# ComparativeGenomicsToolkit/paffy

Measured on AMD Instinct MI355X. Metric: PAF records/sec (shatter+invert+trim pipe); % HBM roofline at 1/2/4/8 GPU, higher is better.
Workload: dtype u8/int64 (float32 identity predicate); 1 GPU; cfg3: 10M synthetic PAF records, mean 2k cigar ops, invert | trim | shatter; pipe=invert|trim|shatter, pipeline_contexts=2, stream_records=10000000, mean_cigar_ops=2048

## Files before the change

### paffy_amd/csrc/flat_kernel.h

```cpp
#ifndef PAFFY_FLAT_KERNEL_H_
#define PAFFY_FLAT_KERNEL_H_

#define FLAT_TILE 1024u
#define FLAT_TILE_SHIFT 10u
#define FLAT_CHUNK_PIECES 4u
#define FLAT_P_CAP 512u
#define FLAT_NO_CHUNK 0xffffffffu
#define FLAT_F_IRREG 1u
#define FLAT_F_NONPLAIN 2u

struct PieceSum {
    uint32_t cnt;
    uint32_t m, x;
    uint32_t ins, del;
    uint32_t rows;
    uint32_t extra;
    uint32_t text_end;
};
static_assert(sizeof(PieceSum) == 32, "two 16-byte stores");

struct FlatParams {
    const uint8_t *in;
    uint32_t in_len;
    const RecMeta *meta;
    const uint32_t *chunk_rec;
    uint32_t n_chunk_slots;
    const uint16_t *nd;
    PieceSum *sums;
    uint32_t *ops_mirror;
    DevInfo *info;
    uint32_t items_mode;
};

__device__ __forceinline__ uint32_t nondigit16(const uint4 &v) {
    const uint32_t w[4] = {v.x, v.y, v.z, v.w};
    uint32_t m = 0;
#pragma unroll
    for (int j = 0; j < 4; j++) {
        uint32_t nd = nondigit4(w[j]) >> 7;
        nd = (nd | (nd >> 7) | (nd >> 14) | (nd >> 21)) & 0xfu;
        m |= nd << (4 * j);
    }
    return m;
}
__device__ __forceinline__ uint32_t wave_fold_u32(uint32_t x) {
    x += dpp_mov_u32<DPP_ROW_SHR(1), 0xf, 0xf>(x);
    x += dpp_mov_u32<DPP_ROW_SHR(2), 0xf, 0xf>(x);
    x += dpp_mov_u32<DPP_ROW_SHR(4), 0xf, 0xf>(x);
    x += dpp_mov_u32<DPP_ROW_SHR(8), 0xf, 0xf>(x);
    x += dpp_mov_u32<DPP_BCAST15, 0xa, 0xf>(x);
    x += dpp_mov_u32<DPP_BCAST31, 0xc, 0xf>(x);
    return x;
}
__device__ __forceinline__ uint32_t wave_sum_u32(uint32_t v) { return wave_last_u32(wave_fold_u32(v)); }
__device__ __forceinline__ void wave_sum6_u32(uint32_t (&x)[6]) {
#define FLAT_FOLD_STEP(CTRL, RM)                                                  \
    _Pragma("unroll") for (int k = 0; k < 6; k++) x[k] += dpp_mov_u32<CTRL, RM, 0xf>(x[k]);
    FLAT_FOLD_STEP(DPP_ROW_SHR(1), 0xf)
    FLAT_FOLD_STEP(DPP_ROW_SHR(2), 0xf)
    FLAT_FOLD_STEP(DPP_ROW_SHR(4), 0xf)
    FLAT_FOLD_STEP(DPP_ROW_SHR(8), 0xf)
    FLAT_FOLD_STEP(DPP_BCAST15, 0xa)
    FLAT_FOLD_STEP(DPP_BCAST31, 0xc)
#undef FLAT_FOLD_STEP
#pragma unroll
    for (int k = 0; k < 6; k++) x[k] = wave_last_u32(x[k]);
}
__device__ __forceinline__ uint32_t uni(uint32_t x) { return (uint32_t)__builtin_amdgcn_readfirstlane((int)x); }
__device__ __forceinline__ uint32_t lane_val(uint32_t x, uint32_t l) { return (uint32_t)__builtin_amdgcn_readlane((int)x, (int)l); }

#define FLAT_PARSE_LDS (16u + FLAT_TILE + 2u * FLAT_P_CAP)
#define FLAT_PARSE_WAVES 4u
template <uint32_t MODE>
__global__ __launch_bounds__(64 * FLAT_PARSE_WAVES) void k_flat_parse(FlatParams F) {
    __shared__ __attribute__((aligned(16))) uint8_t smem[FLAT_PARSE_WAVES][FLAT_PARSE_LDS];
    const uint32_t lane = threadIdx.x & 63u, wave = uni(threadIdx.x >> 6);
    uint8_t *T = smem[wave];
    uint16_t *Pl = reinterpret_cast<uint16_t *>(T + 16u + FLAT_TILE);
    const uint32_t n_waves = gridDim.x * FLAT_PARSE_WAVES;
    for (uint32_t c = blockIdx.x * FLAT_PARSE_WAVES + wave; c < F.n_chunk_slots; c += n_waves) {
        const uint32_t rec = F.chunk_rec[c];
        if (rec == FLAT_NO_CHUNK) continue;
        const uint32_t cg_off = F.meta[rec].cg_off, cg_end = cg_off + F.meta[rec].cg_len;
        const uint32_t tile_first = cg_off >> FLAT_TILE_SHIFT;
        const uint32_t np = ((cg_end - 1u) >> FLAT_TILE_SHIFT) - tile_first + 1u;
        const uint32_t p0 = (c - ((tile_first >> 2) + rec)) * FLAT_CHUNK_PIECES, p1 = p0 + FLAT_CHUNK_PIECES < np ? p0 + FLAT_CHUNK_PIECES : np;
        PieceSum *const rec_sums = F.sums + (tile_first + rec);
        uint32_t tile = tile_first + p0;
        __builtin_amdgcn_wave_barrier();
        if (lane == 0) {
            uint4 h = make_uint4(0, 0, 0, 0);
            if (tile > 0) h = *reinterpret_cast<const uint4 *>(F.in + ((size_t)tile << FLAT_TILE_SHIFT) - 16u);
            *reinterpret_cast<uint4 *>(T) = h;
        }
        __builtin_amdgcn_wave_barrier();
        uint32_t n = 0;
        int32_t prev;
        uint32_t text_end = 0;
        if (p0 == 0) {
            prev = (int32_t)cg_off - 1 - (int32_t)(tile << FLAT_TILE_SHIFT);
        } else {
            uint32_t cnt = 0;
            {
                const uint32_t g = (tile_first << FLAT_TILE_SHIFT) + lane * 16u;
                uint4 v = make_uint4(0x30303030u, 0x30303030u, 0x30303030u, 0x30303030u);
                if (g < F.in_len) v = *reinterpret_cast<const uint4 *>(F.in + g);
                const uint32_t lo_b = cg_off > g ? (cg_off - g < 16u ? cg_off - g : 16u) : 0u;
                cnt = (uint32_t)__popc(nondigit16(v) & 0xffffu & ~((1u << lo_b) - 1u));
            }
            for (uint32_t t = tile_first + 1u + lane; t < tile; t += 64u) cnt += F.nd[t];
            n = wave_sum_u32(cnt);
            const uint4 h = *reinterpret_cast<const uint4 *>(T);
            const uint32_t hm = nondigit16(h);
            prev = hm ? (int32_t)(31 - __clz((int)hm)) - 16 : -17;
            text_end = (uint32_t)((int32_t)(tile << FLAT_TILE_SHIFT) + prev + 1 - (int32_t)cg_off);
        }
        uint16_t *dst = reinterpret_cast<uint16_t *>(F.ops_mirror + (cg_off >> 1));
        for (uint32_t p = p0; p < p1; p++, tile++) {
            const uint32_t t0 = tile << FLAT_TILE_SHIFT, g = t0 + lane * 16u;
            uint4 v = make_uint4(0, 0, 0, 0);
            if (g < F.in_len) v = *reinterpret_cast<const uint4 *>(F.in + g);
            *reinterpret_cast<uint4 *>(T + 16u + lane * 16u) = v;
            const uint32_t ndm = nondigit16(v);
            const uint32_t lo_b = cg_off > g ? (cg_off - g < 16u ? cg_off - g : 16u) : 0u;
            const uint32_t hi_b = cg_end < g + 16u ? (cg_end > g ? cg_end - g : 0u) : 16u;
            uint32_t opmask = ndm & (hi_b >= 16u ? 0xffffu : ((1u << hi_b) - 1u)) & ~((1u << lo_b) - 1u);
            uint32_t bad = (hi_b > lo_b && g + hi_b == cg_end && !((ndm >> (hi_b - 1u)) & 1u)) ? 1u : 0u;
            const uint32_t cnt = (uint32_t)__popc(opmask), inc = wave_incl_scan_u32(cnt), total = wave_last_u32(inc);
            uint32_t rank = inc - cnt;
            while (opmask) {
                const uint32_t j = (uint32_t)__ffs((int)opmask) - 1u;
                opmask &= opmask - 1u;
                if (rank < FLAT_P_CAP) Pl[rank] = (uint16_t)(lane * 16u + j);
                rank++;
            }
            if (total > FLAT_P_CAP) bad = 1u;
            __builtin_amdgcn_wave_barrier();
            const uint32_t top = total < FLAT_P_CAP ? total : FLAT_P_CAP;
            uint32_t acc_mx = 0, acc_id = 0, acc_re = 0, nonplain = 0;
            uint32_t before_first = (uint32_t)prev;
            for (uint32_t i = lane; i < top; i += 64u) {
                const uint32_t pos = Pl[i];
                const uint32_t before = (uint32_t)__builtin_amdgcn_update_dpp((int)before_first, (int)pos, 0x138 , 0xf, 0xf, false);
                before_first = lane_val(pos, 63);
                const uint32_t k = pos - before - 1u;
                const uint32_t a = 12u + pos, sh = a & 3u;
                const uint32_t *wp = reinterpret_cast<const uint32_t *>(T + (a - sh));
                const uint32_t d0 = wp[0], d1 = wp[1];
                const uint32_t hi = __builtin_amdgcn_alignbyte(d1, d0, sh);
                const uint32_t ch = (d1 >> (8u * sh)) & 0xffu;
                const uint32_t kk = k < 4u ? k : 4u;
                const uint32_t x = kk ? ((hi ^ 0x30303030u) & (0xffffffffu << (32u - 8u * kk))) : 0u;
                const uint32_t pr = ((x << 3) + (x << 1) + (x >> 8)) & 0x00ff00ffu;
                const uint32_t len = __umul24(pr & 0xffu, 100u) + (pr >> 16);
                const uint32_t dl = ch - 0x3du;
                const bool known = dl < 28u && ((0x08011081u >> dl) & 1u);
                const uint32_t code = (0x04001023u >> (dl & 0x1cu)) & 7u;
                const bool lead0 = kk >= 2u && ((hi >> (8u * (4u - kk))) & 0xffu) == (uint32_t)'0';
                bad |= ((k - 1u > 3u) | (len - 1u >= 8191u) | lead0 | !known) ? 1u : 0u;
                dst[n + i] = (uint16_t)((len << 3) | code);
                const uint32_t l16 = len & 0xffffu;
                acc_mx += l16 << (((0x16u >> code) & 1u) << 4);
                acc_id += (code == (uint32_t)OP_I ? l16 : 0u) + (code == (uint32_t)OP_D ? l16 << 16 : 0u);
                if (MODE == 2u) acc_re += (code == (uint32_t)OP_M ? 1u : 0u) + (code == (uint32_t)OP_I ? 1u << 16 : 0u);
                else acc_re += code == (uint32_t)OP_M ? 1u + ((MODE == 1u ? (len + 15u) >> 4 : kk - 1u) << 16) : 0u;
                nonplain |= code > (uint32_t)OP_D ? 1u : 0u;
            }
            uint32_t sums6[6] = {acc_mx & 0xffffu, acc_mx >> 16, acc_id & 0xffffu, acc_id >> 16, acc_re & 0xffffu, acc_re >> 16};
            wave_sum6_u32(sums6);
            const uint32_t s_m = sums6[0], s_x = sums6[1], s_i = sums6[2], s_d = sums6[3], s_r = sums6[4], s_e = sums6[5];
            const uint32_t flags = (__any(bad != 0) ? FLAT_F_IRREG : 0u) | (__any(nonplain != 0) ? FLAT_F_NONPLAIN : 0u);
            if (total) {
                const int32_t last = (int32_t)Pl[top - 1u];
                text_end = t0 + (uint32_t)last + 1u - cg_off;
                prev = last - (int32_t)FLAT_TILE;
            } else {
                prev -= (int32_t)FLAT_TILE;
                if (prev < -64) prev = -64;
            }
            if (lane == 0) {
                uint4 *o = reinterpret_cast<uint4 *>(rec_sums + p);
                o[0] = make_uint4(total | (flags << 16), s_m, s_x, s_i);
                o[1] = make_uint4(s_d, s_r, s_e, text_end);
            }
            n += total;
            __builtin_amdgcn_wave_barrier();
            if (lane == 63u) *reinterpret_cast<uint4 *>(T) = v;
            __builtin_amdgcn_wave_barrier();
        }
    }
}


struct FlatSizeParams {
    KParams P;
    PieceSum *sums;
    uint8_t *flat_done;
    uint32_t *defer;
};

struct FlatPre {
    uint32_t cnt, m, x, ins, del, rows, extra, text;
};
__device__ __forceinline__ FlatPre flat_sub(const FlatPre &a, const FlatPre &b) {
    FlatPre r;
    r.cnt = a.cnt - b.cnt; r.m = a.m - b.m; r.x = a.x - b.x; r.ins = a.ins - b.ins; r.del = a.del - b.del;
    r.rows = a.rows - b.rows; r.extra = a.extra - b.extra; r.text = a.text - b.text;
    return r;
}
__device__ __forceinline__ uint32_t flat_ld(const uint32_t *p) { return __hip_atomic_load(p, __ATOMIC_RELAXED, __HIP_MEMORY_SCOPE_AGENT); }

struct FlatRec {
    const PieceSum *ps;
    uint32_t np, n_ops;
    bool in_regs;
    FlatPre inc;
    const uint16_t *ops;
    bool want_text;
    bool extra_icount;

    __device__ __forceinline__ FlatPre piece_prefix(uint32_t j) const {
        FlatPre r;
        r.cnt = r.m = r.x = r.ins = r.del = r.rows = r.extra = r.text = 0;
        if (j == 0) return r;
        if (in_regs) {
            const uint32_t l = j - 1u;
            r.cnt = lane_val(inc.cnt, l); r.m = lane_val(inc.m, l); r.x = lane_val(inc.x, l); r.ins = lane_val(inc.ins, l);
            r.del = lane_val(inc.del, l); r.rows = lane_val(inc.rows, l); r.extra = lane_val(inc.extra, l); r.text = lane_val(inc.text, l);
        } else {
            const uint32_t *q = reinterpret_cast<const uint32_t *>(ps + (j - 1u));
            r.cnt = uni(flat_ld(q)); r.m = uni(flat_ld(q + 1)); r.x = uni(flat_ld(q + 2)); r.ins = uni(flat_ld(q + 3));
            r.del = uni(flat_ld(q + 4)); r.rows = uni(flat_ld(q + 5)); r.extra = uni(flat_ld(q + 6)); r.text = uni(flat_ld(q + 7));
        }
        return r;
    }
    __device__ __forceinline__ uint32_t piece_of(uint32_t r) const {
        if (in_regs) {
            const uint32_t lane = threadIdx.x & 63u;
            return (uint32_t)__popcll(__ballot(lane < np && inc.cnt <= r));
        }
        uint32_t lo = 0, hi = np;
        while (lo < hi) {
            const uint32_t mid = (lo + hi) >> 1;
            if (uni(flat_ld(&ps[mid].cnt)) <= r) lo = mid + 1u;
            else hi = mid;
        }
        return lo;
    }
    __device__ __forceinline__ FlatPre raw_prefix(uint32_t r) const {
        if (r >= n_ops) return piece_prefix(np);
        const uint32_t pc = piece_of(r);
        FlatPre a = piece_prefix(pc);
        if (a.cnt == r) return a;
        const uint32_t lane = threadIdx.x & 63u;
        uint32_t sm = 0, sx = 0, si = 0, sd = 0, sr = 0, se = 0, st = 0;
        for (uint32_t i = a.cnt + lane; i < r; i += 64u) {
            const uint32_t w = ops[i], len = w >> 3, code = w & 7u;
            const uint32_t is_m = 0u - ((0x9u >> code) & 1u);
            const uint32_t dg = (len >= 10u) + (len >= 100u) + (len >= 1000u);
            sm += len & is_m;
            sx += len & ~is_m;
            si += code == (uint32_t)OP_I ? len : 0u;
            sd += code == (uint32_t)OP_D ? len : 0u;
            sr += code == (uint32_t)OP_M ? 1u : 0u;
            se += extra_icount ? (code == (uint32_t)OP_I ? 1u : 0u) : (code == (uint32_t)OP_M ? dg : 0u);
            st += dg + 2u;
        }
        uint32_t sums6[6] = {sm, sx, si, sd, sr, se};
        wave_sum6_u32(sums6);
        a.m += sums6[0]; a.x += sums6[1]; a.ins += sums6[2]; a.del += sums6[3];
        a.rows += sums6[4]; a.extra += sums6[5];
        if (want_text) a.text += wave_sum_u32(st);
        a.cnt = r;
        return a;
    }
};

struct FlatView {
    uint32_t lo, n;
    bool rev, swp;
    FlatPre wlo, whi;
    uint32_t cut_m = 0, cut_x = 0;
    __device__ __forceinline__ uint32_t tm() const { return whi.m - wlo.m - cut_m; }
    __device__ __forceinline__ uint32_t tx() const { return whi.x - wlo.x - cut_x; }
    __device__ __forceinline__ uint32_t ins_v() const { return swp ? whi.del - wlo.del : whi.ins - wlo.ins; }
    __device__ __forceinline__ uint32_t del_v() const { return swp ? whi.ins - wlo.ins : whi.del - wlo.del; }
    __device__ __forceinline__ int64_t tq() const { return (int64_t)tm() + (int64_t)tx() - (int64_t)del_v(); }
    __device__ __forceinline__ int64_t tt() const { return (int64_t)tm() + (int64_t)tx() - (int64_t)ins_v(); }
};

struct FlatState {
    int64_t qlen, qs, qe, tlen, ts, te;
    bool same;
};
__device__ __forceinline__ void flat_invert(FlatState &s) {
    int64_t t;
    t = s.qs; s.qs = s.ts; s.ts = t;
    t = s.qe; s.qe = s.te; s.te = t;
    t = s.qlen; s.qlen = s.tlen; s.tlen = t;
}
__device__ __forceinline__ int flat_check(const FlatState &s, const FlatView &v) {
    if (s.qs < 0 || s.qs >= s.qlen) return PAFFY_ERR_CHECK_QSTART;
    if (s.qs > s.qe || s.qe > s.qlen) return PAFFY_ERR_CHECK_QEND;
    if (s.ts < 0 || s.ts >= s.tlen) return PAFFY_ERR_CHECK_TSTART;
    if (s.ts > s.te || s.te > s.tlen) return PAFFY_ERR_CHECK_TEND;
    if (v.tq() != s.qe - s.qs) return PAFFY_ERR_CHECK_CIGAR_Q;
    if (v.tt() != s.te - s.ts) return PAFFY_ERR_CHECK_CIGAR_T;
    return 0;
}

__device__ __forceinline__ bool flat_filter_pass(const KParams &P, const RecMeta &m, const FlatView &v) {
    const int64_t mm = v.tm(), mx = v.tx();
    const int64_t all = mm + mx;
    const int64_t ins = all - v.tt(), del = all - v.tq();
    const double identity = ratio_f32(mm, mm + (mx - ins - del));
    const double identity_with_gaps = ratio_f32(mm, all);
    const int64_t f_as = P.filter.min_alignment_score, f_cs = P.filter.min_chain_score, f_tl = P.filter.max_tile_level;
    const double f_id = P.filter.min_identity, f_idg = P.filter.min_identity_with_gaps;
    return m.score >= f_as && m.chain_score >= f_cs && (f_tl == -1 || m.tile_level <= f_tl) && identity >= f_id && identity_with_gaps >= f_idg;
}
__device__ __forceinline__ void flat_dropped(const KParams &P, uint8_t *flat_done, uint32_t rec) {
    RecPlan *dp = static_cast<RecPlan *>(P.rec_plan) + rec;
    flat_done[rec] = 1;
    P.status[rec] = (uint32_t)KLASS_LDS << 16;
    P.err_aux[rec] = 0;
    P.n_ops[rec] = 0;
    P.out_len[rec] = 0;
    P.out_rows[rec] = 0;
    dp->flags = 128u;
    dp->n = 0;
}

__device__ __forceinline__ void flat_stats(const KParams &P, uint32_t rec, const FlatView &v) {
    const uint32_t n_i = v.whi.extra - v.wlo.extra, n_other = (v.whi.cnt - v.wlo.cnt) - (v.whi.rows - v.wlo.rows);
    const uint32_t n_d = n_other - n_i;
    int64_t *o = P.rec_stats + 6ull * rec;
    o[0] = (int64_t)v.tm();
    o[1] = (int64_t)v.tx() - (int64_t)(v.whi.ins - v.wlo.ins) - (int64_t)(v.whi.del - v.wlo.del);
    o[2] = (int64_t)(v.swp ? n_d : n_i);
    o[3] = (int64_t)(v.swp ? n_i : n_d);
    o[4] = (int64_t)v.ins_v();
    o[5] = (int64_t)v.del_v();
}
__device__ __forceinline__ bool flat_ratio_lt(uint32_t num, uint32_t den, float thr_f, double thr) {
    const float nf = __uint2float_rn(num), df = __uint2float_rn(den);
    const float p = __fmul_rn(thr_f, df);
    if (nf < __fmul_rn(p, 0.999996f)) return true;
    if (nf > __fmul_rn(p, 1.000004f)) return false;
    return (double)__fdiv_rn(nf, df) < thr;
}
__device__ __forceinline__ bool flat_ratio_ge(uint32_t num, uint32_t den, float id_f, double idd) {
    const float nf = __uint2float_rn(num), df = __uint2float_rn(den);
    const float p = __fmul_rn(id_f, df);
    if (nf > __fmul_rn(p, 1.000004f)) return true;
    if (nf < __fmul_rn(p, 0.999996f)) return false;
    return (double)__fdiv_rn(nf, df) >= idd;
}

__device__ __forceinline__ void flat_trim_prefix(const FlatRec &R, FlatState &s, FlatView &v, float thr_f, float id_f, int64_t max_trim) {
    const double thr = (double)thr_f, idd = (double)id_f;
    const uint32_t lane = threadIdx.x & 63u;
    const uint32_t w_end = v.lo + v.n;
    const uint32_t nb = (R.np + 63u) >> 6;
    int32_t trim_idx = -1;
    uint32_t hit_m = 0, hit_x = 0;
    for (uint32_t bi = 0; bi < nb && trim_idx < 0; bi++) {
        const uint32_t b = v.rev ? bi : nb - 1u - bi;
        const uint32_t p = b * 64u + lane;
        uint32_t a_cnt = 0, a_m = 0, a_x = 0, b_cnt = 0, b_m = 0, b_x = 0;
        if (p < R.np) {
            if (R.in_regs) {
                b_cnt = R.inc.cnt; b_m = R.inc.m; b_x = R.inc.x;
            } else {
                const uint32_t *q = reinterpret_cast<const uint32_t *>(R.ps + p);
                b_cnt = flat_ld(q); b_m = flat_ld(q + 1); b_x = flat_ld(q + 2);
            }
        }
        if (R.in_regs) {
            a_cnt = dpp_mov_u32<0x138, 0xf, 0xf>(b_cnt); a_m = dpp_mov_u32<0x138, 0xf, 0xf>(b_m); a_x = dpp_mov_u32<0x138, 0xf, 0xf>(b_x);
        } else if (p > 0 && p < R.np) {
            const uint32_t *q = reinterpret_cast<const uint32_t *>(R.ps + (p - 1u));
            a_cnt = flat_ld(q); a_m = flat_ld(q + 1); a_x = flat_ld(q + 2);
        }
        if (a_cnt < v.lo) { a_cnt = v.lo; a_m = v.wlo.m; a_x = v.wlo.x; }
        if (a_cnt > w_end) { a_cnt = w_end; a_m = v.whi.m; a_x = v.whi.x; }
        if (b_cnt < v.lo) { b_cnt = v.lo; b_m = v.wlo.m; b_x = v.wlo.x; }
        if (b_cnt > w_end) { b_cnt = w_end; b_m = v.whi.m; b_x = v.whi.x; }
        const bool live = p < R.np && b_cnt > a_cnt;
        const uint32_t c_m = v.rev ? v.whi.m - b_m : a_m - v.wlo.m, c_x = v.rev ? v.whi.x - b_x : a_x - v.wlo.x;
        const uint32_t chunk_x = b_x - a_x;
        const bool may_hit = live && !(c_m > 0 && (double)c_m >= thr * 1.00001 * (double)(c_m + c_x + chunk_x)) &&
                             !(max_trim >= 0 && (int64_t)c_m + (int64_t)c_x > max_trim);
        unsigned long long flagged = __ballot(may_hit);
        while (flagged) {
            const uint32_t t = v.rev ? (uint32_t)__ffsll((long long)flagged) - 1u : 63u - (uint32_t)__clzll((long long)flagged);
            flagged &= ~(1ull << t);
            const uint32_t ra = lane_val(a_cnt, t), rb = lane_val(b_cnt, t);
            uint32_t pm = lane_val(c_m, t), px = lane_val(c_x, t);
            const uint32_t x_end = px + lane_val(chunk_x, t);
            const uint32_t vb = v.rev ? w_end - rb : ra - v.lo, ve = v.rev ? w_end - ra : rb - v.lo;
            int32_t hit = -1;
            for (uint32_t i0 = vb; i0 < ve; i0 += 64u) {
                if (i0 != vb && pm > 0 && (double)pm >= thr * 1.00001 * (double)(pm + x_end)) break;
                const uint32_t i = i0 + lane;
                uint32_t len = 0, code = 0;
                if (i < ve) {
                    const uint32_t w = R.ops[v.rev ? w_end - 1u - i : v.lo + i];
                    len = w >> 3;
                    code = w & 7u;
                }
                const uint32_t is_m = 0u - ((0x9u >> code) & 1u);
                const uint32_t im = wave_incl_scan_u32(len & is_m), ix = wave_incl_scan_u32(len & ~is_m);
                const uint32_t cm = pm + im, cx = px + ix;
                const bool ok = i < ve && !(max_trim >= 0 && (int64_t)(cm + cx) > max_trim) && flat_ratio_lt(cm, cm + cx, thr_f, thr);
                const unsigned long long hb = __ballot(ok);
                if (hb) {
                    const uint32_t hl = 63u - (uint32_t)__clzll((long long)hb);
                    hit = (int32_t)(i0 + hl);
                    hit_m = lane_val(cm, hl);
                    hit_x = lane_val(cx, hl);
                }
                pm += wave_last_u32(im);
                px += wave_last_u32(ix);
            }
            if (hit >= 0) {
                trim_idx = hit;
                break;
            }
        }
    }
    if (trim_idx < 0) return;
    uint32_t best = 0xffffffffu;
    {
        uint32_t pm = 0, px = 0;
        for (uint32_t i0 = 0; i0 <= (uint32_t)trim_idx && best == 0xffffffffu; i0 += 64u) {
            const uint32_t i = i0 + lane;
            uint32_t len = 0, code = 0;
            if (i <= (uint32_t)trim_idx) {
                const uint32_t w = R.ops[v.rev ? w_end - 1u - i : v.lo + i];
                len = w >> 3;
                code = w & 7u;
            }
            const uint32_t is_m = 0u - ((0x9u >> code) & 1u);
            const uint32_t vm = len & is_m, vx = len & ~is_m;
            const uint32_t im = wave_incl_scan_u32(vm), ix = wave_incl_scan_u32(vx);
            const uint32_t sm = hit_m - (pm + im - vm), sx = hit_x - (px + ix - vx);
            const bool ok = i <= (uint32_t)trim_idx && flat_ratio_ge(sm, sm + sx, id_f, idd);
            const unsigned long long hb = __ballot(ok);
            if (hb) best = i0 + (uint32_t)__ffsll((long long)hb) - 1u;
            pm += wave_last_u32(im);
            px += wave_last_u32(ix);
        }
    }
    const uint32_t count = best != 0xffffffffu ? best : (uint32_t)trim_idx + 1u;
    if (count == 0) return;
    const int64_t old_tt = v.tt(), old_tq = v.tq();
    {
        const FlatPre cut = R.raw_prefix(v.rev ? v.lo + v.n - count : v.lo + count);
        if (v.rev) {
            v.whi = cut;
        } else {
            v.wlo = cut;
            v.lo += count;
        }
    }
    v.n -= count;
    const int64_t d_t = old_tt - v.tt(), d_q = old_tq - v.tq();
    s.ts += d_t;
    if (s.same) s.qs += d_q;
    else s.qe -= d_q;
}

#define FLAT_F_ROW_PIECES 0x200000u
#define FLAT_F_COPY 0x400000u
#define FLAT_COPY_MAX (1u << 18)
#define FLAT_ROW_PIECES_BYTES 144u
// ... 947 lines not shown
```

Baseline: 24.72 million records/s.

## Rewrite flat-parse CIGAR decode with udot4 digit math and LDS-absolute op positions

Replaces the per-byte nondigit mask fold with udot4 dot products, and stores absolute LDS byte addresses in the op-position list so the previous op position is read from memory instead of a DPP shift plus readlane. CIGAR length decoding uses udot4. Validity checks are OR-accumulated into three bitmasks and tested once after the loop. Per-op accumulators are trimmed: the X sum is rebuilt as I+D, and =/X ops go through a wave-uniform slow path with a separate reduction. The position list grows to a full tile and output stores use global address-space pointers. This cuts VALU work in the decode loop, at the cost of more LDS and subtle invariants about address encoding and validity equivalence.

```diff
diff --git a/paffy_amd/csrc/flat_kernel.h b/paffy_amd/csrc/flat_kernel.h
--- a/paffy_amd/csrc/flat_kernel.h
+++ b/paffy_amd/csrc/flat_kernel.h
@@ -32,16 +32,11 @@
     uint32_t items_mode;
 };
 
+__device__ __forceinline__ uint32_t udot4(uint32_t x, uint32_t w, uint32_t a) { return __builtin_amdgcn_udot4(x, w, a, false); }
 __device__ __forceinline__ uint32_t nondigit16(const uint4 &v) {
-    const uint32_t w[4] = {v.x, v.y, v.z, v.w};
-    uint32_t m = 0;
-#pragma unroll
-    for (int j = 0; j < 4; j++) {
-        uint32_t nd = nondigit4(w[j]) >> 7;
-        nd = (nd | (nd >> 7) | (nd >> 14) | (nd >> 21)) & 0xfu;
-        m |= nd << (4 * j);
-    }
-    return m;
+    const uint32_t lo = udot4(nondigit4(v.y), 0x80402010u, udot4(nondigit4(v.x), 0x08040201u, 0u));
+    const uint32_t hi = udot4(nondigit4(v.w), 0x80402010u, udot4(nondigit4(v.z), 0x08040201u, 0u));
+    return (hi << 1) | (lo >> 7);
 }
 __device__ __forceinline__ uint32_t wave_fold_u32(uint32_t x) {
     x += dpp_mov_u32<DPP_ROW_SHR(1), 0xf, 0xf>(x);
@@ -53,9 +48,10 @@
     return x;
 }
 __device__ __forceinline__ uint32_t wave_sum_u32(uint32_t v) { return wave_last_u32(wave_fold_u32(v)); }
-__device__ __forceinline__ void wave_sum6_u32(uint32_t (&x)[6]) {
+template <int N>
+__device__ __forceinline__ void wave_sums_u32(uint32_t (&x)[N]) {
 #define FLAT_FOLD_STEP(CTRL, RM)                                                  \
-    _Pragma("unroll") for (int k = 0; k < 6; k++) x[k] += dpp_mov_u32<CTRL, RM, 0xf>(x[k]);
+    _Pragma("unroll") for (int k = 0; k < N; k++) x[k] += dpp_mov_u32<CTRL, RM, 0xf>(x[k]);
     FLAT_FOLD_STEP(DPP_ROW_SHR(1), 0xf)
     FLAT_FOLD_STEP(DPP_ROW_SHR(2), 0xf)
     FLAT_FOLD_STEP(DPP_ROW_SHR(4), 0xf)
@@ -64,19 +60,27 @@
     FLAT_FOLD_STEP(DPP_BCAST31, 0xc)
 #undef FLAT_FOLD_STEP
 #pragma unroll
-    for (int k = 0; k < 6; k++) x[k] = wave_last_u32(x[k]);
-}
+    for (int k = 0; k < N; k++) x[k] = wave_last_u32(x[k]);
+}
+__device__ __forceinline__ void wave_sum6_u32(uint32_t (&x)[6]) { wave_sums_u32<6>(x); }
 __device__ __forceinline__ uint32_t uni(uint32_t x) { return (uint32_t)__builtin_amdgcn_readfirstlane((int)x); }
 __device__ __forceinline__ uint32_t lane_val(uint32_t x, uint32_t l) { return (uint32_t)__builtin_amdgcn_readlane((int)x, (int)l); }
 
-#define FLAT_PARSE_LDS (16u + FLAT_TILE + 2u * FLAT_P_CAP)
+#define FLAT_P_SLOTS FLAT_TILE
+#define FLAT_PARSE_PL (16u + FLAT_TILE + 16u)
+#define FLAT_PARSE_LDS (FLAT_PARSE_PL + 2u * FLAT_P_SLOTS)
 #define FLAT_PARSE_WAVES 4u
+#define FLAT_CODE_TAB 0x34770127u
+#define FLAT_CODE_LETTERS_LO 0x3d44494du
+#define FLAT_CODE_LETTERS_HI 0xffffff58u
 template <uint32_t MODE>
 __global__ __launch_bounds__(64 * FLAT_PARSE_WAVES) void k_flat_parse(FlatParams F) {
     __shared__ __attribute__((aligned(16))) uint8_t smem[FLAT_PARSE_WAVES][FLAT_PARSE_LDS];
     const uint32_t lane = threadIdx.x & 63u, wave = uni(threadIdx.x >> 6);
+    uint8_t *const L = &smem[0][0];
     uint8_t *T = smem[wave];
-    uint16_t *Pl = reinterpret_cast<uint16_t *>(T + 16u + FLAT_TILE);
+    const uint32_t ebase = wave * FLAT_PARSE_LDS + 12u;
+    const uint32_t pl0 = wave * FLAT_PARSE_LDS + FLAT_PARSE_PL;
     const uint32_t n_waves = gridDim.x * FLAT_PARSE_WAVES;
     for (uint32_t c = blockIdx.x * FLAT_PARSE_WAVES + wave; c < F.n_chunk_slots; c += n_waves) {
         const uint32_t rec = F.chunk_rec[c];
@@ -115,7 +119,9 @@
             prev = hm ? (int32_t)(31 - __clz((int)hm)) - 16 : -17;
             text_end = (uint32_t)((int32_t)(tile << FLAT_TILE_SHIFT) + prev + 1 - (int32_t)cg_off);
         }
-        uint16_t *dst = reinterpret_cast<uint16_t *>(F.ops_mirror + (cg_off >> 1));
+        const uintptr_t dst = reinterpret_cast<uintptr_t>(F.ops_mirror + (cg_off >> 1)) - (uintptr_t)(pl0 - 2u);
+        typedef __attribute__((address_space(1))) uint8_t *GlobalBytes;
+        typedef __attribute__((address_space(1))) uint16_t *GlobalWord;
         for (uint32_t p = p0; p < p1; p++, tile++) {
             const uint32_t t0 = tile << FLAT_TILE_SHIFT, g = t0 + lane * 16u;
             uint4 v = make_uint4(0, 0, 0, 0);
@@ -127,51 +133,71 @@
             uint32_t opmask = ndm & (hi_b >= 16u ? 0xffffu : ((1u << hi_b) - 1u)) & ~((1u << lo_b) - 1u);
             uint32_t bad = (hi_b > lo_b && g + hi_b == cg_end && !((ndm >> (hi_b - 1u)) & 1u)) ? 1u : 0u;
             const uint32_t cnt = (uint32_t)__popc(opmask), inc = wave_incl_scan_u32(cnt), total = wave_last_u32(inc);
-            uint32_t rank = inc - cnt;
-            while (opmask) {
-                const uint32_t j = (uint32_t)__ffs((int)opmask) - 1u;
-                opmask &= opmask - 1u;
-                if (rank < FLAT_P_CAP) Pl[rank] = (uint16_t)(lane * 16u + j);
-                rank++;
+            {
+                uint32_t w = pl0 + 2u * (inc - cnt);
+                const uint32_t e0 = ebase + lane * 16u;
+                for (; opmask; opmask &= opmask - 1u, w += 2u) *reinterpret_cast<uint16_t *>(L + w) = (uint16_t)(e0 + (uint32_t)__builtin_ctz(opmask));
+                if (lane == 0) *reinterpret_cast<int16_t *>(L + pl0 - 2u) = (int16_t)((int32_t)ebase + (prev < -17 ? -17 : prev));
             }
             if (total > FLAT_P_CAP) bad = 1u;
             __builtin_amdgcn_wave_barrier();
             const uint32_t top = total < FLAT_P_CAP ? total : FLAT_P_CAP;
-            uint32_t acc_mx = 0, acc_id = 0, acc_re = 0, nonplain = 0;
-            uint32_t before_first = (uint32_t)prev;
-            for (uint32_t i = lane; i < top; i += 64u) {
-                const uint32_t pos = Pl[i];
-                const uint32_t before = (uint32_t)__builtin_amdgcn_update_dpp((int)before_first, (int)pos, 0x138 , 0xf, 0xf, false);
-                before_first = lane_val(pos, 63);
-                const uint32_t k = pos - before - 1u;
-                const uint32_t a = 12u + pos, sh = a & 3u;
-                const uint32_t *wp = reinterpret_cast<const uint32_t *>(T + (a - sh));
-                const uint32_t d0 = wp[0], d1 = wp[1];
-                const uint32_t hi = __builtin_amdgcn_alignbyte(d1, d0, sh);
-                const uint32_t ch = (d1 >> (8u * sh)) & 0xffu;
-                const uint32_t kk = k < 4u ? k : 4u;
-                const uint32_t x = kk ? ((hi ^ 0x30303030u) & (0xffffffffu << (32u - 8u * kk))) : 0u;
-                const uint32_t pr = ((x << 3) + (x << 1) + (x >> 8)) & 0x00ff00ffu;
-                const uint32_t len = __umul24(pr & 0xffu, 100u) + (pr >> 16);
-                const uint32_t dl = ch - 0x3du;
-                const bool known = dl < 28u && ((0x08011081u >> dl) & 1u);
-                const uint32_t code = (0x04001023u >> (dl & 0x1cu)) & 7u;
-                const bool lead0 = kk >= 2u && ((hi >> (8u * (4u - kk))) & 0xffu) == (uint32_t)'0';
-                bad |= ((k - 1u > 3u) | (len - 1u >= 8191u) | lead0 | !known) ? 1u : 0u;
-                dst[n + i] = (uint16_t)((len << 3) | code);
-                const uint32_t l16 = len & 0xffffu;
-                acc_mx += l16 << (((0x16u >> code) & 1u) << 4);
-                acc_id += (code == (uint32_t)OP_I ? l16 : 0u) + (code == (uint32_t)OP_D ? l16 << 16 : 0u);
-                if (MODE == 2u) acc_re += (code == (uint32_t)OP_M ? 1u : 0u) + (code == (uint32_t)OP_I ? 1u << 16 : 0u);
-                else acc_re += code == (uint32_t)OP_M ? 1u + ((MODE == 1u ? (len + 15u) >> 4 : kk - 1u) << 16) : 0u;
-                nonplain |= code > (uint32_t)OP_D ? 1u : 0u;
-            }
-            uint32_t sums6[6] = {acc_mx & 0xffffu, acc_mx >> 16, acc_id & 0xffffu, acc_id >> 16, acc_re & 0xffffu, acc_re >> 16};
-            wave_sum6_u32(sums6);
-            const uint32_t s_m = sums6[0], s_x = sums6[1], s_i = sums6[2], s_d = sums6[3], s_r = sums6[4], s_e = sums6[5];
-            const uint32_t flags = (__any(bad != 0) ? FLAT_F_IRREG : 0u) | (__any(nonplain != 0) ? FLAT_F_NONPLAIN : 0u);
+            uint32_t v_len = 0, v_dig = 0, v_let = 0;
+            uint32_t acc_m = 0;
+            uint32_t acc_id = 0;
+            uint32_t acc_r = 0;
+            uint32_t acc_eq = 0, acc_xx = 0;
+            uint32_t eqx = 0;
+            const uint32_t a_end = pl0 - 2u + 2u * top;
+            const GlobalBytes tile_dst = (GlobalBytes)(dst + 2u * (uintptr_t)n);
+            for (uint32_t a = pl0 - 2u + 2u * lane; a < a_end; a += 128u) {
+                const uint32_t before = (uint32_t)(int32_t)*reinterpret_cast<const int16_t *>(L + a);
+                const uint32_t pos = *reinterpret_cast<const uint16_t *>(L + a + 2u);
+                const uint32_t first = L[before + 5u], ch = L[pos + 4u];
+                const uint32_t km1 = pos - before - 2u;
+                const uint32_t dig = (km1 << 3) + 7u;
+                const uint32_t *wp = reinterpret_cast<const uint32_t *>(L + (pos & ~3u));
+                const uint32_t hi = __builtin_amdgcn_alignbyte(wp[1], wp[0], pos & 3u);
+                const uint32_t x = (hi ^ 0x30303030u) & (uint32_t)((int32_t)0x80000000 >> (dig & 31u));
+                const uint32_t len = udot4(x, 0x010a0000u, __umul24(udot4(x, 0x0000010au, 0u), 100u));
+                const uint32_t sel = ch & 0x1cu;
+                const uint32_t code = (FLAT_CODE_TAB >> sel) & 7u;
+                v_let |= __builtin_amdgcn_perm(FLAT_CODE_LETTERS_HI, FLAT_CODE_LETTERS_LO, code) ^ ch;
+                v_len |= len | (first - 0x31u);
+                v_dig |= dig;
+                *(GlobalWord)(tile_dst + a) = (uint16_t)((len << 3) | code);
+                const bool is_m = sel == 0x0cu;
+                acc_m += is_m ? len + ((MODE == 0u ? km1 : MODE == 1u ? (len + 15u) >> 4 : 0u) << 16) : 0u;
+                acc_r += (is_m ? 1u : 0u) + (MODE == 2u ? ((0x100u >> sel) & 1u) << 16 : 0u);
+                acc_id += __umul24(len, (0x00100100u >> sel) & 0x10001u);
+                if (__any(sel >= 0x18u)) {
+                    asm volatile("");
+                    acc_eq += sel == 0x1cu ? len : 0u;
+                    acc_xx += sel == 0x18u ? len : 0u;
+                    eqx = 1u;
+                }
+            }
+            const bool nonplain = __any(eqx != 0);
+            bad |= (v_len >= 8192u || v_dig > 31u || (v_let & 0xffu)) ? 1u : 0u;
+            uint32_t s_m, s_x, s_i, s_d, s_r, s_e;
+            if (MODE == 1u) {
+                uint32_t s[5] = {acc_m & 0xffffu, acc_m >> 16, acc_id & 0xffffu, acc_id >> 16, acc_r};
+                wave_sums_u32<5>(s);
+                s_m = s[0]; s_e = s[1]; s_i = s[2]; s_d = s[3]; s_r = s[4];
+            } else {
+                uint32_t s[4] = {acc_m & 0xffffu, acc_id & 0xffffu, acc_id >> 16, MODE == 2u ? acc_r : (acc_m & 0xffff0000u) | acc_r};
+                wave_sums_u32<4>(s);
+                s_m = s[0]; s_i = s[1]; s_d = s[2]; s_r = s[3] & 0xffffu; s_e = s[3] >> 16;
+            }
+            s_x = s_i + s_d;
+            if (nonplain) {
+                uint32_t s[2] = {acc_eq, acc_xx};
+                wave_sums_u32<2>(s);
+                s_m += s[0]; s_x += s[1];
+            }
+            const uint32_t flags = (__any(bad != 0) ? FLAT_F_IRREG : 0u) | (nonplain ? FLAT_F_NONPLAIN : 0u);
             if (total) {
-                const int32_t last = (int32_t)Pl[top - 1u];
+                const int32_t last = (int32_t)uni(*reinterpret_cast<const uint16_t *>(L + pl0 + 2u * (top - 1u))) - (int32_t)ebase;
                 text_end = t0 + (uint32_t)last + 1u - cg_off;
                 prev = last - (int32_t)FLAT_TILE;
             } else {
```

After: 26.23 million records/s, median of 6. 6.1% higher.
